# una-dinosauria/local-search-quantization

Hardware: AMD Instinct MI355X
Metric: vectors encoded/sec (ICM, m=8 h=256) (higher is better)
Workload: dtype f32

## Files before the change

### local-search-quantization_amd/csrc/lsq_icm.hip

```cpp
#include <stdlib.h>

#include <mutex>
#include <type_traits>

#include "lsq_wave.h"
#include "lsq_xload.h"
#include <atomic>

namespace {

template <int M, int SL, int ABL = 0, int DEPTH = 2, int NT = 1024>
__global__ __launch_bounds__(NT) void icm_walk_kernel(const float *__restrict__ U, const float *__restrict__ Ts, const float *__restrict__ T,
                                                        uint8_t *__restrict__ rec, unsigned short *__restrict__ valid,
                                                        int64_t n, const WalkNodes nodes, int per_pass, int use_skip, int direct_max,
                                                        unsigned long long *__restrict__ active_total,
                                                        const uint8_t *__restrict__ ref_rec, const unsigned short *__restrict__ ref_valid,
                                                        const int *__restrict__ idle_if_set) {
    constexpr int CS = (M <= 8) ? 8 : 16;
    constexpr int NS = LSQ_H / SL;
    if (idle_if_set && *idle_if_set) return;
    constexpr int LPV = SL / 4;
    constexpr int VPW = 64 / LPV;
    constexpr int CW = (M - 1 + 3) / 4;
    constexpr int RW = CS / 4;
// ... 140 lines not shown
            try_phase(std::integral_constant<int, 0>{}); try_phase(std::integral_constant<int, 1>{});
            try_phase(std::integral_constant<int, 2>{}); try_phase(std::integral_constant<int, 3>{});
            try_phase(std::integral_constant<int, 4>{}); try_phase(std::integral_constant<int, 5>{});
            try_phase(std::integral_constant<int, 6>{}); try_phase(std::integral_constant<int, 7>{});
        }
        __syncthreads();
    };

    const int64_t npass = (n + per_pass - 1) / per_pass;
    for (int64_t pass = blockIdx.x; pass < npass; pass += gridDim.x) {
        const int64_t lo = pass * per_pass;
        const int64_t hi = (lo + per_pass < n) ? lo + per_pass : n;
        const int cnt = (int)(hi - lo);

        for (int nu = 0; nu < nodes.count; ++nu) {
        const int j = nodes.j[nu];
        const float *__restrict__ Usj = U + (int64_t)j * n * LSQ_H;
        {
            const int base = (int)threadIdx.x * EPT;
            int f[EPT], c = 0;
#pragma unroll
            for (int e = 0; e < EPT; ++e) {
                const int idx = base + e;
                f[e] = 0;
                if (idx < cnt) f[e] = (!use_skip) || !((valid[lo + idx] >> j) & 1);
                c += f[e];
            }
            int inc = c;
#pragma unroll
            for (int off = 1; off < 64; off <<= 1) {
                const int t = __shfl_up(inc, off, 64);
                if (lane >= off) inc += t;
            }
            if (lane == 63) wave_tot[wave] = inc;
            __syncthreads();
            int wbase = 0;
            for (int w2 = 0; w2 < wave; ++w2) wbase += wave_tot[w2];
            int pos = wbase + inc - c;
#pragma unroll
            for (int e = 0; e < EPT; ++e)
                if (f[e]) list[pos++] = (unsigned short)(base + e);
            if (threadIdx.x == NT - 1) nact_s = wbase + inc;
            __syncthreads();
        }
        const int nact = nact_s;
        if (nact == 0) { __syncthreads(); continue; }
        if (threadIdx.x == 0) {
            stat_s[0] += (unsigned)nact;
            stat_s[nact <= direct_max ? 2 : 1] += 1u;
            stat_s[4 + ((nodes.pos0 + nu) & (LSQ_WALK_TRACE - 1))] += (unsigned)nact;
        }
        if (nact <= direct_max) {
            const float *__restrict__ Tj = T + (int64_t)j * M * LSQ_H * LSQ_H;
            constexpr int LB = LSQ_LIGHT_LB(M);
            for (int r0 = wave; r0 < nact; r0 += NW * LB) {
                int64_t vi[LB];
                bool on[LB];
#pragma unroll
                for (int e = 0; e < LB; ++e) {
                    const int r = r0 + e * NW;
                    on[e] = r < nact;
                    vi[e] = lo + __builtin_amdgcn_readfirstlane((int)list[on[e] ? r : r0]);
                }
                light_update<M, CS, LB>(rec, valid, ref_rec, ref_valid, Usj, Tj, n, SL, j, vi, on, lane);
            }
            __syncthreads();
            continue;
        }
        for (int ci = threadIdx.x; ci < nact; ci += NT) best64[ci] = ~0ull;

        walk_slices(j, lo, nact, nact == cnt, 0, NS);
        {
            constexpr int EPD = (PP + NT - 1) / NT;
            int64_t vi[EPD];
            uint32_t vcode[EPD];
            bool von[EPD];
#pragma unroll
            for (int e = 0; e < EPD; ++e) {
                const int ci = (int)threadIdx.x + e * NT;
                von[e] = ci < nact;
                vi[e] = lo + (von[e] ? list[ci] : 0);
                vcode[e] = von[e] ? (uint32_t)(best64[ci] & 0xffffffffull) : 0u;
            }
            apply_node_results<CS, EPD>(rec, valid, vi, vcode, von, j, ref_rec, ref_valid);
        }
        __syncthreads();
        }
    }
    __syncthreads();
    if (active_total)
        for (int e = threadIdx.x; e < 4 + LSQ_WALK_TRACE; e += NT)
            if (stat_s[e]) atomicAdd(active_total + e, (unsigned long long)stat_s[e]);
}

template <int SL>
__global__ __launch_bounds__(256) void tables_to_slices_kernel(const float *__restrict__ T, float *__restrict__ Ts, int m) {
    constexpr int NS = LSQ_H / SL, LPV = SL / 4;
    const int64_t total = (int64_t)m * NS * (m - 1) * LSQ_H * LPV;
    const int64_t e = (int64_t)blockIdx.x * 256 + threadIdx.x;
    if (e >= total) return;
    const int qq = (int)(e % LPV);
    int64_t r = e / LPV;
    const int b = (int)(r % LSQ_H); r /= LSQ_H;
    const int kk = (int)(r % (m - 1)); r /= (m - 1);
    const int slice = (int)(r % NS);
    const int j = (int)(r / NS);
    const int k = kk + (kk >= j ? 1 : 0);
    reinterpret_cast<f32x4 *>(Ts)[e] =
        *reinterpret_cast<const f32x4 *>(T + (((int64_t)j * m + k) * LSQ_H + b) * LSQ_H + slice * SL + qq * 4);
}

template <int M>
__global__ __launch_bounds__(256) void icm_wave_kernel(const float *__restrict__ U, const float *__restrict__ T, uint8_t *__restrict__ rec,
                                                       unsigned short *__restrict__ valid, int64_t n, const WalkNodes nodes, int SL, int use_skip,
                                                       unsigned long long *__restrict__ active_total, const uint8_t *__restrict__ ref_rec,
                                                       const unsigned short *__restrict__ ref_valid, const int *__restrict__ idle_if_set) {
    constexpr int CS = (M <= 8) ? 8 : 16;
    constexpr int LB = LSQ_LIGHT_LB(M);
    if (idle_if_set && *idle_if_set) return;
    __shared__ unsigned stat_s[4 + LSQ_WALK_TRACE];
    for (int e = threadIdx.x; e < 4 + LSQ_WALK_TRACE; e += 256) stat_s[e] = 0u;
    __syncthreads();
    const int lane = threadIdx.x & 63;
    const int64_t wv = (int64_t)blockIdx.x * 4 + __builtin_amdgcn_readfirstlane((int)(threadIdx.x >> 6));
    const int64_t i0 = wv * LB;
    const int LPV = SL / 4;
    const bool have_ref = ref_rec && ref_valid;
    CodeRec cr[LB], rr[LB];
    uint32_t vm[LB], rv[LB];
    bool on[LB];
#pragma unroll
    for (int e = 0; e < LB; ++e) {
        on[e] = i0 + e < n;
        cr[e].lo = cr[e].hi = rr[e].lo = rr[e].hi = 0ull;
        vm[e] = rv[e] = 0u;
        if (on[e]) {
            cr[e] = load_rec<CS>(rec, i0 + e);
            if (valid) vm[e] = (uint32_t)__builtin_amdgcn_readfirstlane((int)valid[i0 + e]);
            if (have_ref) {
                rr[e] = load_rec<CS>(ref_rec, i0 + e);
                rv[e] = (uint32_t)__builtin_amdgcn_readfirstlane((int)ref_valid[i0 + e]);
            }
        }
    }
    unsigned total = 0, wave_nodes = 0;
    for (int nu = 0; nu < nodes.count; ++nu) {
        const int j = nodes.j[nu];
        bool need[LB];
        unsigned cnt = 0;
#pragma unroll
        for (int e = 0; e < LB; ++e) {
            need[e] = on[e] && (!use_skip || !((vm[e] >> j) & 1u));
            cnt += need[e] ? 1u : 0u;
        }
        if (cnt == 0) continue;
        const float *__restrict__ Usj = U + (int64_t)j * n * LSQ_H;
        const float *__restrict__ Tj = T + (int64_t)j * M * LSQ_H * LSQ_H;
        f32x4 s[LB], c[LB][M > 1 ? M - 1 : 1];
#pragma unroll
        for (int e = 0; e < LB; ++e) {
            s[e] = (f32x4){0.f, 0.f, 0.f, 0.f};
            if (need[e]) s[e] = (reinterpret_cast<const f32x4 *>(Usj + ((int64_t)(lane / LPV) * n + (i0 + e)) * SL))[lane % LPV];
        }
#pragma unroll
        for (int e = 0; e < LB; ++e)
            if (need[e]) {
#pragma unroll
                for (int kk = 0; kk < M - 1; ++kk) {
                    const int k = kk + (kk >= j ? 1 : 0);
                    c[e][kk] = reinterpret_cast<const f32x4 *>(Tj + ((int64_t)(k * LSQ_H) + cr[e].get(k)) * LSQ_H)[lane];
                }
            }
#pragma unroll
        for (int e = 0; e < LB; ++e)
            if (need[e]) {
#pragma unroll
                for (int kk = 0; kk < M - 1; ++kk) s[e] = s[e] + c[e][kk];
                const uint32_t code = (uint32_t)wave_first_argmin(s[e], lane);
                if (code != cr[e].get(j)) { cr[e].set(j, code); vm[e] = 1u << j; }
                else vm[e] |= 1u << j;
                if (have_ref && cr[e].lo == rr[e].lo && (CS == 8 || cr[e].hi == rr[e].hi)) vm[e] |= rv[e];
            }
        total += cnt;
        ++wave_nodes;
        if (lane == 0) atomicAdd(&stat_s[4 + ((nodes.pos0 + nu) & (LSQ_WALK_TRACE - 1))], cnt);
    }
#pragma unroll
    for (int e = 0; e < LB; ++e)
        if (on[e] && lane == 0) {
            *reinterpret_cast<uint64_t *>(rec + (i0 + e) * CS) = cr[e].lo;
            if (CS == 16) *reinterpret_cast<uint64_t *>(rec + (i0 + e) * CS + 8) = cr[e].hi;
            if (valid) valid[i0 + e] = (unsigned short)vm[e];
        }
    if (lane == 0) { atomicAdd(&stat_s[0], total); atomicAdd(&stat_s[2], wave_nodes); }
    __syncthreads();
    if (active_total)
        for (int e = threadIdx.x; e < 4 + LSQ_WALK_TRACE; e += 256)
            if (stat_s[e]) atomicAdd(active_total + e, (unsigned long long)stat_s[e]);
}

__device__ inline bool perturb_record(uint64_t (&w)[2], int m, int npert, uint64_t seed, uint32_t it, uint64_t gi) {
    int need = npert < m ? npert : m;
    bool changed = false;
    for (int g = 0; 4 * g < m && need > 0; ++g) {
        const lsq_u32x4 sel = lsq_rng_block(seed, gi, it, LSQ_DOM_PERTURB, (uint32_t)g);
        const lsq_u32x4 vals = lsq_rng_block(seed, gi, it, LSQ_DOM_PERTURB, (uint32_t)(4 + g));
#pragma unroll
        for (int e = 0; e < 4; ++e) {
            const int pp = 4 * g + e;
            if (pp < m && need > 0 && lsq_mulhi32(sel.v[e], (uint32_t)(m - pp)) < (uint32_t)need) {
                const uint64_t val = lsq_mulhi32(vals.v[e], LSQ_H);
                const int sh = 8 * (pp & 7);
                changed |= (((w[pp >> 3] >> sh) & 0xffull) != val);
                w[pp >> 3] = (w[pp >> 3] & ~(0xffull << sh)) | (val << sh);
                --need;
            }
        }
    }
    return changed;
}

template <int CS>
__device__ inline void perturb_next_store(const lsq_perturb_next &pn, int64_t i, const uint32_t (&fin)[CS / 4], unsigned short vfin) {
    uint64_t w[2];
    w[0] = (uint64_t)fin[0] | ((uint64_t)fin[1] << 32);
    w[1] = (CS == 16) ? ((uint64_t)fin[CS / 4 - 2] | ((uint64_t)fin[CS / 4 - 1] << 32)) : 0ull;
#ifdef LSQ_TUNING
    if (pn.abl & 16) return;
    const bool changed = (pn.abl & 1) ? false : perturb_record(w, pn.m, pn.npert, pn.seed, pn.it, pn.goff + (uint64_t)i);
#else
    const bool changed = perturb_record(w, pn.m, pn.npert, pn.seed, pn.it, pn.goff + (uint64_t)i);
#endif
    uint64_t *q = reinterpret_cast<uint64_t *>(pn.dst + i * CS);
    q[0] = w[0];
    if (CS == 16) q[1] = w[1];
    if (pn.vdst) pn.vdst[i] = changed ? (unsigned short)0 : vfin;
}

template <int CS>
__global__ __launch_bounds__(256) void perturb_kernel(const uint8_t *__restrict__ src, uint8_t *__restrict__ dst, int64_t n,
                                                      int m, int npert, uint64_t seed, uint32_t it, uint64_t goff,
                                                      const unsigned short *__restrict__ vsrc, unsigned short *__restrict__ vdst) {
    const int64_t i = (int64_t)blockIdx.x * blockDim.x + threadIdx.x;
    if (i >= n) return;
    uint64_t w[2];
    const uint64_t *p = reinterpret_cast<const uint64_t *>(src + i * CS);
    w[0] = p[0];
    w[1] = (CS == 16) ? p[1] : 0ull;
    const bool changed = perturb_record(w, m, npert, seed, it, goff + (uint64_t)i);
    uint64_t *q = reinterpret_cast<uint64_t *>(dst + i * CS);
    q[0] = w[0];
    if (CS == 16) q[1] = w[1];
    if (vdst) vdst[i] = changed ? (unsigned short)0 : vsrc[i];
}

template <int VW>
__device__ inline int load_start(int c, int lp, int s) { return c + 16 * VW * s + VW * lp; }
template <int VW, typename OFF>
__device__ inline f32x4 load4(const float *p, OFF off, int c, int lp, int d) {
    if constexpr (VW == 4) {
        const int t = load_start<VW>(c, lp, 0);
        return *reinterpret_cast<const f32x4 *>(p + (size_t)(off + (OFF)(t < d ? t : 0)));
    }
    f32x4 v;
#pragma unroll
    for (int s = 0; s < 4; ++s) {
        const int t = load_start<VW>(c, lp, s);
        v[s] = p[(size_t)(off + (OFF)(t < d ? t : 0))];
    }
    return v;
}

template <class XT, int VW> struct XQuad { f32x4 v; __device__ f32x4 get() const { return v; } };
template <> struct XQuad<uint8_t, 4> { uint32_t w; __device__ f32x4 get() const { return lsq_widen4(w); } };
template <> struct XQuad<uint8_t, 1> {
    uint32_t b[4];
    __device__ f32x4 get() const { return (f32x4){(float)b[0], (float)b[1], (float)b[2], (float)b[3]}; }
};
template <int VW>
__device__ inline XQuad<float, VW> xquad_load(const float *x, int c, int lp, int d) { return XQuad<float, VW>{load4<VW>(x, 0, c, lp, d)}; }
template <int VW>
__device__ inline XQuad<uint8_t, VW> xquad_load(const uint8_t *x, int c, int lp, int d) {
    XQuad<uint8_t, VW> q;
    if constexpr (VW == 4) {
        const int t = load_start<VW>(c, lp, 0);
        q.w = lsq_ld4_packed(x + (t < d ? t : 0));
    } else {
#pragma unroll
        for (int s = 0; s < 4; ++s) {
            const int t = load_start<VW>(c, lp, s);
            q.b[s] = x[t < d ? t : 0];
        }
    }
    return q;
}

__device__ inline float row_sum16(float v) {
    v = v + dpp_self<DPP_XOR1, 0xf>(v);
    v = v + dpp_self<DPP_XOR2, 0xf>(v);
    v = v + dpp_self<DPP_HALF_MIRROR, 0xf>(v);
    return v + dpp_self<DPP_MIRROR, 0xf>(v);
}

template <int M, int MODE, int HASV, int NQ, int VW, class XT = float>
__device__ inline void cost4_body(const XT *__restrict__ X, const float *__restrict__ K,
                                  const uint8_t *rec, uint8_t *cur, float *__restrict__ prev,
                                  unsigned long long *__restrict__ counters, int64_t n, int64_t w, int64_t nwaves, int d,
                                  const unsigned short *vnew, unsigned short *vcur, const lsq_perturb_next &pn) {
    static_assert(VW == 4 || VW == 1, "load width: 16 or 4 bytes");
    using koff_t = std::conditional_t<VW == 4, uint32_t, uint64_t>;
    constexpr int CS = (M <= 8) ? 8 : 16;
    constexpr int RW = CS / 4;
    const int lane = threadIdx.x & 63;
    const int qtr = lane >> 4, lp = lane & 15;
    unsigned n_eq = 0, n_lt = 0;
    for (int64_t base = w * 64; base < n; base += nwaves * 64) {
        const int64_t il = base + lane;
        const bool livel = il < n;
        const int64_t ic = livel ? il : n - 1;
        uint32_t rn[RW], cw[RW];
        float pl = 0.0f;
        unsigned short vc = 0, vn = 0;
        {
            const uint32_t *rp = reinterpret_cast<const uint32_t *>(rec + ic * CS), *cp = reinterpret_cast<const uint32_t *>(cur + ic * CS);
#pragma unroll
            for (int q = 0; q < RW; ++q) rn[q] = rp[q];
            if (MODE == 1) {
#pragma unroll
                for (int q = 0; q < RW; ++q) cw[q] = cp[q];
                pl = prev[ic];
            }
            if (HASV) vc = vcur[ic];
            if (HASV && MODE == 1) vn = vnew[ic];
        }
        bool same = (MODE == 1);
#pragma unroll
        for (int q = 0; q < RW; ++q) {
            if (MODE == 0) cw[q] = rn[q];
            same = same && (rn[q] == cw[q]);
        }
        const bool skip = livel && same && (pl == pl);
        const unsigned nskip = (unsigned)__popcll(__ballot(skip));
        if (lane == 0) n_eq += nskip;
        unsigned short vfin = vc;
        const bool merge_v = HASV && MODE == 1 && same && livel;
        if (merge_v) vfin = (unsigned short)(vfin | vn);
        uint64_t accepted = 0;
        float newp = 0.0f;
        uint64_t todo = __ballot(livel && !skip);
#ifdef LSQ_TUNING
        if (pn.abl & 8) todo = 0;
#endif
        int nsidx[4];
        bool nhv[4];
        auto pick = [&]() {
#pragma unroll
            for (int v = 0; v < 4; ++v) {
                nhv[v] = todo != 0;
                nsidx[v] = nhv[v] ? __builtin_ctzll(todo) : (v ? nsidx[0] : 0);
                if (nhv[v]) todo &= todo - 1;
            }
        };
        auto xrow = [&]() -> const XT * {
            const int mys = qtr == 0 ? nsidx[0] : qtr == 1 ? nsidx[1] : qtr == 2 ? nsidx[2] : nsidx[3];
            return X + (base + mys) * (int64_t)d;
        };
        XQuad<XT, VW> xn[NQ];
        auto xload = [&](const XT *x, int c0) {
#pragma unroll
            for (int g = 0; g < NQ; ++g) {
                xn[g] = xquad_load<VW>(x, c0 + 64 * g, lp, d);
            }
        };
        pick();
        const XT *xnext = xrow();
        if (nhv[0]) xload(xnext, 0);
        while (nhv[0]) {
            int sidx[4];
            bool hv[4];
#pragma unroll
            for (int v = 0; v < 4; ++v) { sidx[v] = nsidx[v]; hv[v] = nhv[v]; }
            const XT *x = xnext;
            pick();
            xnext = xrow();
            const bool live = qtr == 0 ? hv[0] : qtr == 1 ? hv[1] : qtr == 2 ? hv[2] : hv[3];
            uint32_t r[RW];
            float pc;
            {
                uint32_t rv4[4][RW];
                float pc4[4];
#pragma unroll
                for (int v = 0; v < 4; ++v) {
#pragma unroll
                    for (int q = 0; q < RW; ++q) rv4[v][q] = (uint32_t)__builtin_amdgcn_readlane((int)rn[q], sidx[v]);
                    pc4[v] = __int_as_float(__builtin_amdgcn_readlane(__float_as_int(pl), sidx[v]));
                }
#pragma unroll
                for (int q = 0; q < RW; ++q) r[q] = qtr == 0 ? rv4[0][q] : qtr == 1 ? rv4[1][q] : qtr == 2 ? rv4[2][q] : rv4[3][q];
                pc = qtr == 0 ? pc4[0] : qtr == 1 ? pc4[1] : qtr == 2 ? pc4[2] : pc4[3];
            }
            koff_t kb[M];
#pragma unroll
            for (int k = 0; k < M; ++k) kb[k] = ((koff_t)(k * LSQ_H) + (koff_t)((r[k >> 2] >> (8 * (k & 3))) & 0xffu)) * (koff_t)d;
            f32x4 p = (f32x4){0.f, 0.f, 0.f, 0.f};
            for (int c0 = 0; c0 < d; c0 += 64 * NQ) {
                f32x4 xv[NQ], kv[NQ][M];
                bool ok[NQ][4];
#pragma unroll
                for (int g = 0; g < NQ; ++g) {
                    const int c = c0 + 64 * g;
#pragma unroll
                    for (int e = 0; e < 4; ++e) ok[g][e] = load_start<VW>(c, lp, e / VW) < d;
                    xv[g] = xn[g].get();
#pragma unroll
                    for (int k = 0; k < M; ++k) kv[g][k] = load4<VW>(K, kb[k], c, lp, d);
                }
                if (c0 + 64 * NQ < d) xload(x, c0 + 64 * NQ);
                else xload(xnext, 0);
#pragma unroll
                for (int g = 0; g < NQ; ++g) {
                    f32x4 cb = (f32x4){0.f, 0.f, 0.f, 0.f};
#pragma unroll
                    for (int k = 0; k < M; ++k) cb = cb + kv[g][k];
                    const f32x4 rr = cb - xv[g];
                    const f32x4 sq = rr * rr;
                    p.x = p.x + (ok[g][0] ? sq.x : 0.0f);
                    p.y = p.y + (ok[g][1] ? sq.y : 0.0f);
                    p.z = p.z + (ok[g][2] ? sq.z : 0.0f);
                    p.w = p.w + (ok[g][3] ? sq.w : 0.0f);
                }
            }
            float cost;
            if constexpr (VW == 4) cost = row_sum16((p.x + p.y) + (p.z + p.w));
            else cost = (row_sum16(p.x) + row_sum16(p.y)) + (row_sum16(p.z) + row_sum16(p.w));
#pragma unroll
            for (int v2 = 0; v2 < 4; ++v2) {
                const float cv = __int_as_float(__builtin_amdgcn_readlane(__float_as_int(cost), 16 * v2));
                if (hv[v2] && lane == sidx[v2]) newp = cv;
            }
            if (MODE == 1) {
                const bool eq = live && (cost == pc), lt = live && (cost < pc);
                const uint64_t bl = __ballot(lt && lp == 0);
                const unsigned ne = (unsigned)__popcll(__ballot(eq && lp == 0)), nl = (unsigned)__popcll(bl);
#pragma unroll
                for (int v2 = 0; v2 < 4; ++v2)
                    if ((bl >> (16 * v2)) & 1ull) accepted |= 1ull << sidx[v2];
                if (lane == 0) { n_eq += ne; n_lt += nl; }
            }
        }
        const bool acc = (accepted >> lane) & 1ull;
        if (MODE == 0) {
            if (livel) prev[il] = newp;
        } else if (acc) {
            prev[il] = newp;
            uint32_t *qd = reinterpret_cast<uint32_t *>(cur + il * CS);
#pragma unroll
            for (int q = 0; q < RW; ++q) qd[q] = rn[q];
        }
        if (HASV && MODE == 1 && (acc || merge_v)) vcur[il] = acc ? vn : vfin;
        if (pn.on && livel) {
            uint32_t fin[RW];
#pragma unroll
            for (int q = 0; q < RW; ++q) fin[q] = acc ? rn[q] : cw[q];
            perturb_next_store<CS>(pn, il, fin, acc ? vn : vfin);
        }
    }
    if (MODE == 1) {
        __shared__ unsigned cnt_s[2];
        if (threadIdx.x == 0) { cnt_s[0] = 0u; cnt_s[1] = 0u; }
        __syncthreads();
        if (lane == 0 && n_eq) atomicAdd(&cnt_s[0], n_eq);
        if (lane == 0 && n_lt) atomicAdd(&cnt_s[1], n_lt);
        __syncthreads();
        if (threadIdx.x == 0 && cnt_s[0]) atomicAdd(&counters[0], (unsigned long long)cnt_s[0]);
        if (threadIdx.x == 0 && cnt_s[1]) atomicAdd(&counters[1], (unsigned long long)cnt_s[1]);
    }
}

template <int M, int MODE, int HASV, int NQ, int VW, class XT = float>
__global__ __launch_bounds__(256) void cost4_kernel(const XT *__restrict__ X, const float *__restrict__ K, const uint8_t *rec, uint8_t *cur,
                                                    float *__restrict__ prev, unsigned long long *__restrict__ counters, int64_t n, int d,
                                                    const unsigned short *vnew, unsigned short *vcur, const lsq_perturb_next pn) {
    cost4_body<M, MODE, HASV, NQ, VW, XT>(X, K, rec, cur, prev, counters, n, __builtin_amdgcn_readfirstlane((int)(blockIdx.x * 4 + (threadIdx.x >> 6))),
                                      (int64_t)gridDim.x * 4, d, vnew, vcur, pn);
}
template <int M, int MODE, int HASV, int NQ, int VW, class XT = float>
__global__ __launch_bounds__(256) __attribute__((amdgpu_waves_per_eu(4, 4))) void cost4w_kernel(const XT *__restrict__ X, const float *__restrict__ K,
                                                    const uint8_t *rec, uint8_t *cur, float *__restrict__ prev,
                                                    unsigned long long *__restrict__ counters, int64_t n, int d,
                                                    const unsigned short *vnew, unsigned short *vcur, const lsq_perturb_next pn) {
    cost4_body<M, MODE, HASV, NQ, VW, XT>(X, K, rec, cur, prev, counters, n, __builtin_amdgcn_readfirstlane((int)(blockIdx.x * 4 + (threadIdx.x >> 6))),
                                      (int64_t)gridDim.x * 4, d, vnew, vcur, pn);
}

__global__ __launch_bounds__(256) void sum_f64_kernel(const float *__restrict__ v, int64_t n, double *__restrict__ sum) {
    __shared__ double sh[4];
    double acc = 0.0;
    for (int64_t i = (int64_t)blockIdx.x * blockDim.x + threadIdx.x; i < n; i += (int64_t)gridDim.x * blockDim.x) acc += (double)v[i];
    for (int off = 32; off > 0; off >>= 1) acc += __shfl_down(acc, off, 64);
    if ((threadIdx.x & 63) == 0) sh[threadIdx.x >> 6] = acc;
    __syncthreads();
    if (threadIdx.x == 0) atomicAdd(sum, sh[0] + sh[1] + sh[2] + sh[3]);
}

template <int CS>
__global__ __launch_bounds__(256) void codes_expand_kernel(const uint8_t *__restrict__ tight, int64_t n, int m, uint8_t *__restrict__ rec) {
    const int64_t i = (int64_t)blockIdx.x * blockDim.x + threadIdx.x;
    if (i >= n) return;
    uint64_t w[2] = {0ull, 0ull};
    for (int j = 0; j < m; ++j) w[j >> 3] |= (uint64_t)tight[i * m + j] << (8 * (j & 7));
    uint64_t *q = reinterpret_cast<uint64_t *>(rec + i * CS);
    q[0] = w[0];
    if (CS == 16) q[1] = w[1];
}
template <int CS>
__global__ __launch_bounds__(256) void codes_compact_kernel(const uint8_t *__restrict__ rec, int64_t n, int m, uint8_t *__restrict__ tight) {
    const int64_t i = (int64_t)blockIdx.x * blockDim.x + threadIdx.x;
    if (i >= n) return;
    for (int j = 0; j < m; ++j) tight[i * m + j] = rec[i * CS + j];
}
template <int CS>
__global__ __launch_bounds__(256) void codes_from_i16_kernel(const int16_t *__restrict__ B, int64_t n, int m, int h,
                                                             uint8_t *__restrict__ rec, int *__restrict__ bad) {
    const int64_t i = (int64_t)blockIdx.x * blockDim.x + threadIdx.x;
    if (i >= n) return;
    uint64_t w[2] = {0ull, 0ull};
    for (int j = 0; j < m; ++j) {
        const int v = (int)B[i * m + j];
        if (v < 1 || v > h) { *bad = 1; continue; }
        w[j >> 3] |= (uint64_t)(v - 1) << (8 * (j & 7));
    }
    uint64_t *q = reinterpret_cast<uint64_t *>(rec + i * CS);
    q[0] = w[0];
    if (CS == 16) q[1] = w[1];
}
template <int CS>
__global__ __launch_bounds__(256) void codes_to_i16_kernel(const uint8_t *__restrict__ rec, int64_t n, int m, int16_t *__restrict__ B) {
    const int64_t i = (int64_t)blockIdx.x * blockDim.x + threadIdx.x;
    if (i >= n) return;
    for (int j = 0; j < m; ++j) B[i * m + j] = (int16_t)(rec[i * CS + j] + 1);
}

__global__ __launch_bounds__(256) void synth_data_u8_kernel(uint64_t seed, uint64_t goff, int64_t n, int d, float *__restrict__ X) {
    const int64_t q = (int64_t)blockIdx.x * blockDim.x + threadIdx.x;
    const int d4 = (d + 3) >> 2;
    if (q >= n * d4) return;
    const int64_t i = q / d4;
    const int t0 = (int)(q % d4) * 4;
    const lsq_u32x4 r = lsq_rng_block(seed, goff + (uint64_t)i, (uint32_t)(t0 >> 10), LSQ_DOM_DATA, (uint32_t)((t0 & 1023) >> 2));
    for (int e = 0; e < 4 && t0 + e < d; ++e) X[i * (int64_t)d + t0 + e] = (float)(r.v[e] >> 24);
}
__global__ __launch_bounds__(256) void randinit_kernel(uint64_t seed, uint64_t goff, int64_t n, int m, int h, uint8_t *__restrict__ tight) {
    const int64_t i = (int64_t)blockIdx.x * blockDim.x + threadIdx.x;
    if (i >= n) return;
    for (int j = 0; j < m; ++j)
        tight[i * m + j] = (uint8_t)lsq_mulhi32(lsq_rng_word(seed, goff + (uint64_t)i, 0, LSQ_DOM_INIT, (uint32_t)j), (uint32_t)h);
}
__global__ __launch_bounds__(256) void synth_codebooks_kernel(uint64_t seed, int m, int h, int d, float *__restrict__ K) {
    const int64_t q = (int64_t)blockIdx.x * blockDim.x + threadIdx.x;
    if (q >= (int64_t)m * h * d) return;
    const int64_t row = q / d;
    const int t = (int)(q % d);
    const uint64_t pick = lsq_rng_word(seed, (uint64_t)row, 0, LSQ_DOM_CODEBOOK, 0);
    const uint32_t w = lsq_rng_word(seed ^ 0x5bd1e995ull, pick, (uint32_t)(t >> 10), LSQ_DOM_DATA, (uint32_t)(t & 1023));
    K[q] = (float)(w >> 24) / (float)m;
}

inline unsigned thread_grid(int64_t n) { return (unsigned)((n + 255) / 256); }

}


template <int M, int SL, int ABL = 0, int DEPTH = 2, int NT = 1024>
static int launch_walk_t(hipStream_t s, const float *U, const float *Ts, const float *T, uint8_t *rec, unsigned short *valid, int64_t n,
                         const WalkNodes &nodes, int use_skip, unsigned long long *active_total, int light,
                         const uint8_t *ref_rec, const unsigned short *ref_valid, const int *idle_if_set) {
    constexpr int TAB = (M - 1) * LSQ_H * (SL / 4);
    constexpr int PP = lsq_walk_pp(M, SL);
    constexpr int LDS_BYTES = TAB * 16 + PP * 8 + PP * 2;
    static_assert(LDS_BYTES + 256 <= 160 * 1024, "slice table + running best must fit the 160 KiB LDS");
    int per_pass = 1, npass = 1;
    lsq_walk_geometry(n, PP, &per_pass, &npass);
    const int direct_max = light >= 0 ? light : LSQ_KNOB("LSQ_WALK_DIRECT", 256);
    const int skip = (use_skip && valid) ? 1 : 0;
    static LdsOptIn optin;
    LSQ_TRY(optin_lds(optin, &icm_walk_kernel<M, SL, ABL, DEPTH, NT>, LDS_BYTES));
    const unsigned grid = (unsigned)(npass < 256 ? npass : 256);
    hipLaunchKernelGGL((icm_walk_kernel<M, SL, ABL, DEPTH, NT>), dim3(grid), dim3(NT), LDS_BYTES, s, U, Ts, T, rec, valid, n, nodes, per_pass,
                       skip, (T && ABL == 0) ? direct_max : 0, active_total, skip ? ref_rec : nullptr, skip ? ref_valid : nullptr, idle_if_set);
    LSQ_HIP(hipGetLastError());
    return LSQ_OK;
}

int lsq_launch_icm_walk(hipStream_t s, const float *U, const float *Ts, const float *T, uint8_t *rec, unsigned short *valid, int64_t n, int m,
                        const int32_t *order, int nnodes, int pos0, int max_per, int use_skip, unsigned long long *active_total, int ablation, int light,
                        const uint8_t *ref_rec, const unsigned short *ref_valid, const int *idle_if_set, int *launched) {
    if (n <= 0 || nnodes <= 0) return LSQ_OK;
    return for_walk_launches(order, nnodes, pos0, m, max_per, launched, [&](const WalkNodes &nodes) -> int {
#define LSQ_WALK_ARGS s, U, Ts, T, rec, valid, n, nodes, use_skip, active_total, light, ref_rec, ref_valid, idle_if_set
#define LSQ_WALK_CASE_MID(MM) case MM: LSQ_TRY((launch_walk_t<MM, 8, 0, 2>(LSQ_WALK_ARGS))); break;
#define LSQ_WALK_CASE_BIG(MM) case MM: LSQ_TRY((launch_walk_t<MM, 8, 0, 4, 512>(LSQ_WALK_ARGS))); break;
#define LSQ_WALK_CASE(MM) case MM: LSQ_TRY((launch_walk_t<MM, 16, 0, 3>(LSQ_WALK_ARGS))); break;
#ifdef LSQ_TUNING
        if (m == 8 && ablation == 1) return launch_walk_t<8, 16, 1>(LSQ_WALK_ARGS);
        if (m == 8 && ablation == 2) return launch_walk_t<8, 16, 2>(LSQ_WALK_ARGS);
        if (m == 8 && ablation == 3) return launch_walk_t<8, 16, 3>(LSQ_WALK_ARGS);
        if (m == 8 && ablation == 4) return launch_walk_t<8, 16, 4>(LSQ_WALK_ARGS);
#else
        (void)ablation;
#endif
        switch (m) {
            LSQ_WALK_CASE(1) LSQ_WALK_CASE(2) LSQ_WALK_CASE(3) LSQ_WALK_CASE(4)
            LSQ_WALK_CASE(5) LSQ_WALK_CASE(6) LSQ_WALK_CASE(7) LSQ_WALK_CASE(8)
            LSQ_WALK_CASE_MID(9) LSQ_WALK_CASE_MID(10) LSQ_WALK_CASE_MID(11) LSQ_WALK_CASE_MID(12)
            LSQ_WALK_CASE_MID(13) LSQ_WALK_CASE_BIG(14) LSQ_WALK_CASE_BIG(15) LSQ_WALK_CASE_BIG(16)
        }
#undef LSQ_WALK_ARGS
#undef LSQ_WALK_CASE
#undef LSQ_WALK_CASE_BIG
#undef LSQ_WALK_CASE_MID
        return LSQ_OK;
    });
}

int lsq_launch_tables_to_slices(hipStream_t s, const float *T, float *Ts, int m, int sl) {
    if (m < 2) return LSQ_OK;
    const int64_t total = (int64_t)m * (LSQ_H / sl) * (m - 1) * LSQ_H * (sl / 4);
    const unsigned grid = (unsigned)((total + 255) / 256);
    if (sl == 16) hipLaunchKernelGGL(tables_to_slices_kernel<16>, dim3(grid), dim3(256), 0, s, T, Ts, m);
    else hipLaunchKernelGGL(tables_to_slices_kernel<8>, dim3(grid), dim3(256), 0, s, T, Ts, m);
    LSQ_HIP(hipGetLastError());
    return LSQ_OK;
}

#define LSQ_CS_LAUNCH(m, KERNEL, GRID, ...)                                                       \
    do {                                                                                           \
        if (lsq_code_stride(m) == 8) hipLaunchKernelGGL(KERNEL<8>, dim3(GRID), dim3(256), 0, s, __VA_ARGS__);  \
        else hipLaunchKernelGGL(KERNEL<16>, dim3(GRID), dim3(256), 0, s, __VA_ARGS__);             \
        LSQ_HIP(hipGetLastError());                                                                \
    } while (0)

int lsq_launch_icm_wave(hipStream_t s, const float *U, const float *T, uint8_t *rec, unsigned short *valid, int64_t n, int m, const int32_t *order,
                        int nnodes, int pos0, int max_per, int use_skip, unsigned long long *active_total, const uint8_t *ref_rec,
                        const unsigned short *ref_valid, int *launched) {
    if (n <= 0 || nnodes <= 0) return LSQ_OK;
    const int skip = (use_skip && valid) ? 1 : 0;
    LSQ_TRY(for_walk_launches(order, nnodes, pos0, m, max_per, launched, [&](const WalkNodes &nodes) -> int {
        const int lb = LSQ_LIGHT_LB(m);
        const unsigned grid = (unsigned)((n + 4 * lb - 1) / (4 * lb));
        LSQ_DISPATCH_M(m, hipLaunchKernelGGL(icm_wave_kernel<M_>, dim3(grid), dim3(256), 0, s, U, T, rec, valid, n, nodes, lsq_walk_slice_width(m), skip,
                                             active_total, skip ? ref_rec : nullptr, skip ? ref_valid : nullptr, static_cast<const int *>(nullptr)));
        return LSQ_OK;
    }));
    LSQ_HIP(hipGetLastError());
    return LSQ_OK;
}

int lsq_launch_perturb(hipStream_t s, const uint8_t *src, uint8_t *dst, int64_t n, int m, int npert, uint64_t seed,
                       uint32_t it, uint64_t global_offset, const unsigned short *vsrc, unsigned short *vdst) {
    if (n <= 0) return LSQ_OK;
    LSQ_CS_LAUNCH(m, perturb_kernel, thread_grid(n), src, dst, n, m, npert, seed, it, global_offset, vsrc, vdst);
    return LSQ_OK;
}

const void *lsq_probe_kernel_icm() { return reinterpret_cast<const void *>(&tables_to_slices_kernel<16>); }

template <int M, int NQ, int VW, class XT>
static void launch_cost_t(hipStream_t s, const XT *X, const float *K, const uint8_t *rec, uint8_t *cur, float *prev,
                          unsigned long long *counters, int64_t n, int d, int mode, const unsigned short *vnew, unsigned short *vcur,
                          const lsq_perturb_next &pn) {
    static std::atomic<int> per_cu_known[3];
    auto launch = [&](auto kern, int which) {
        int per_cu = per_cu_known[which].load(std::memory_order_relaxed);
        if (per_cu == 0) {
            int nb = 0;
            if (hipOccupancyMaxActiveBlocksPerMultiprocessor(&nb, kern, 256, 0) != hipSuccess || nb < 1) nb = 4;
            per_cu = nb > 8 ? 8 : nb;
            per_cu_known[which].store(per_cu, std::memory_order_relaxed);
        }
        const int64_t want = (n + 255) / 256, cap = 256 * (int64_t)per_cu;
        hipLaunchKernelGGL(kern, dim3((unsigned)(want < cap ? want : cap)), dim3(256), 0, s, X, K, rec, cur, prev, counters, n, d, vnew, vcur, pn);
    };
    if constexpr (NQ == 1) {
        if (mode == 1) launch(cost4_kernel<M, 1, 1, 1, VW, XT>, 0); else if (vcur) launch(cost4_kernel<M, 0, 1, 1, VW, XT>, 1); else launch(cost4_kernel<M, 0, 0, 1, VW, XT>, 2);
    } else if constexpr (M <= 8) {
        if (mode == 1) launch(cost4w_kernel<M, 1, 1, 2, VW, XT>, 0); else if (vcur) launch(cost4w_kernel<M, 0, 1, 2, VW, XT>, 1); else launch(cost4w_kernel<M, 0, 0, 2, VW, XT>, 2);
    }
}

template <class XT>
static int launch_cost_x(hipStream_t s, const XT *X, const float *K, const uint8_t *rec, uint8_t *cur, float *prev,
                         unsigned long long *counters, int64_t n, int d, int m, int mode, const unsigned short *vnew, unsigned short *vcur,
                         const lsq_perturb_next *next) {
    if (n <= 0) return LSQ_OK;
    if (mode == 1 && (!vnew || !vcur)) { lsq_set_error("lsq_launch_cost: accept mode needs both validity arrays"); return LSQ_EINVAL; }
    lsq_perturb_next pn = {};
    if (next) pn = *next;
    pn.abl = LSQ_KNOB("LSQ_COST_ABL", 0);
    if (d % 4 == 0 && lsq_x_vec_ok(X) && (uintptr_t)K % 16 == 0) {
        if ((int64_t)m * LSQ_H * d >= (1ll << 31)) { lsq_set_error("lsq_launch_cost: codebook matrix too large"); return LSQ_EINVAL; }
        if (d > 64 && m <= 8) {
            LSQ_DISPATCH_M(m, (launch_cost_t<M_, 2, 4>(s, X, K, rec, cur, prev, counters, n, d, mode, vnew, vcur, pn)));
        } else {
            LSQ_DISPATCH_M(m, (launch_cost_t<M_, 1, 4>(s, X, K, rec, cur, prev, counters, n, d, mode, vnew, vcur, pn)));
        }
    } else {
        LSQ_DISPATCH_M(m, (launch_cost_t<M_, 1, 1>(s, X, K, rec, cur, prev, counters, n, d, mode, vnew, vcur, pn)));
    }
    LSQ_HIP(hipGetLastError());
    return LSQ_OK;
}

int lsq_launch_cost(hipStream_t s, const float *X, const float *K, const uint8_t *rec, uint8_t *cur, float *prev,
                    unsigned long long *counters, int64_t n, int d, int m, int mode, const unsigned short *vnew, unsigned short *vcur,
                    const lsq_perturb_next *next) {
    return launch_cost_x(s, X, K, rec, cur, prev, counters, n, d, m, mode, vnew, vcur, next);
}
int lsq_launch_cost(hipStream_t s, const uint8_t *X, const float *K, const uint8_t *rec, uint8_t *cur, float *prev,
                    unsigned long long *counters, int64_t n, int d, int m, int mode, const unsigned short *vnew, unsigned short *vcur,
                    const lsq_perturb_next *next) {
    return launch_cost_x(s, X, K, rec, cur, prev, counters, n, d, m, mode, vnew, vcur, next);
}

int lsq_launch_sum_f64(hipStream_t s, const float *v, int64_t n, double *sum) {
    if (n <= 0) return LSQ_OK;
    unsigned g = thread_grid(n);
    if (g > 1024) g = 1024;
    hipLaunchKernelGGL(sum_f64_kernel, dim3(g), dim3(256), 0, s, v, n, sum);
    LSQ_HIP(hipGetLastError());
    return LSQ_OK;
}

int lsq_launch_codes_expand(hipStream_t s, const uint8_t *tight, int64_t n, int m, uint8_t *rec) {
    if (n <= 0) return LSQ_OK;
    LSQ_CS_LAUNCH(m, codes_expand_kernel, thread_grid(n), tight, n, m, rec);
    return LSQ_OK;
}
int lsq_launch_codes_compact(hipStream_t s, const uint8_t *rec, int64_t n, int m, uint8_t *tight) {
    if (n <= 0) return LSQ_OK;
    LSQ_CS_LAUNCH(m, codes_compact_kernel, thread_grid(n), rec, n, m, tight);
    return LSQ_OK;
}
int lsq_launch_codes_from_i16(hipStream_t s, const int16_t *B, int64_t n, int m, int h, uint8_t *rec, int *bad_flag) {
    if (n <= 0) return LSQ_OK;
    LSQ_CS_LAUNCH(m, codes_from_i16_kernel, thread_grid(n), B, n, m, h, rec, bad_flag);
    return LSQ_OK;
}
int lsq_launch_codes_to_i16(hipStream_t s, const uint8_t *rec, int64_t n, int m, int16_t *B) {
    if (n <= 0) return LSQ_OK;
    LSQ_CS_LAUNCH(m, codes_to_i16_kernel, thread_grid(n), rec, n, m, B);
    return LSQ_OK;
}

int lsq_launch_synth_data_u8(hipStream_t s, uint64_t seed, uint64_t global_offset, int64_t n, int d, float *X) {
    if (n <= 0) return LSQ_OK;
    const int64_t items = n * ((d + 3) >> 2);
    hipLaunchKernelGGL(synth_data_u8_kernel, dim3(thread_grid(items)), dim3(256), 0, s, seed, global_offset, n, d, X);
    LSQ_HIP(hipGetLastError());
    return LSQ_OK;
}
int lsq_launch_randinit(hipStream_t s, uint64_t seed, uint64_t global_offset, int64_t n, int m, int h, uint8_t *tight) {
    if (n <= 0) return LSQ_OK;
    hipLaunchKernelGGL(randinit_kernel, dim3(thread_grid(n)), dim3(256), 0, s, seed, global_offset, n, m, h, tight);
    LSQ_HIP(hipGetLastError());
    return LSQ_OK;
}
int lsq_launch_synth_codebooks(hipStream_t s, uint64_t seed, int m, int h, int d, float *K) {
    hipLaunchKernelGGL(synth_codebooks_kernel, dim3(thread_grid((int64_t)m * h * d)), dim3(256), 0, s, seed, m, h, d, K);
    LSQ_HIP(hipGetLastError());
    return LSQ_OK;
}
```

Baseline: 21.36 million.

## Add software-pipelined buffer-load cost kernel for m<=8 with cross-row prefetch

Replaces the NQ=2 cost kernel for m<=8 with a new body that uses raw buffer loads with out-of-bounds clamping in place of per-lane bounds checks. It double-buffers codeword and X quads across 64-column chunks and across row groups, and prefetches the next batch's codes, prev costs and validity words while the current batch computes. The aim is to hide memory latency and remove address and predicate arithmetic, at the cost of higher register pressure and more complex control flow. It also applies to d<=64, and shared pre-load and store helpers are factored out.

Result: no change. 21.53 million, median of 2 (+0.8%).

```diff
diff --git a/local-search-quantization_amd/csrc/lsq_icm.hip b/local-search-quantization_amd/csrc/lsq_icm.hip
--- a/local-search-quantization_amd/csrc/lsq_icm.hip
+++ b/local-search-quantization_amd/csrc/lsq_icm.hip
@@ -466,7 +466,66 @@
     return v + dpp_self<DPP_MIRROR, 0xf>(v);
 }
 
-template <int M, int MODE, int HASV, int NQ, int VW, class XT = float>
+template <int RW>
+struct CostPre { uint32_t rn[RW], cw[RW]; float pl; unsigned short vc, vn; };
+template <int RW, int MODE, int HASV>
+__device__ inline void cost_pre_load(CostPre<RW> &q, const uint8_t *rec, const uint8_t *cur, const float *prev, const unsigned short *vnew,
+                                     const unsigned short *vcur, int64_t ic) {
+    const uint32_t *rp = reinterpret_cast<const uint32_t *>(rec + ic * (4 * RW)), *cp = reinterpret_cast<const uint32_t *>(cur + ic * (4 * RW));
+    q.pl = 0.0f;
+    q.vc = 0;
+    q.vn = 0;
+#pragma unroll
+    for (int e = 0; e < RW; ++e) q.rn[e] = rp[e];
+#pragma unroll
+    for (int e = 0; e < RW; ++e) q.cw[e] = (MODE == 1) ? cp[e] : q.rn[e];
+    if (MODE == 1) q.pl = prev[ic];
+    if (HASV) q.vc = vcur[ic];
+    if (HASV && MODE == 1) q.vn = vnew[ic];
+}
+template <int RW, int MODE, int HASV>
+__device__ inline void cost_batch_store(const CostPre<RW> &q, bool livel, int64_t il, bool acc, bool merge_v, unsigned short vfin, float newp,
+                                        uint8_t *cur, float *prev, unsigned short *vcur, const lsq_perturb_next &pn) {
+    if (MODE == 0) {
+        if (livel) prev[il] = newp;
+    } else if (acc) {
+        prev[il] = newp;
+        uint32_t *qd = reinterpret_cast<uint32_t *>(cur + il * (4 * RW));
+#pragma unroll
+        for (int e = 0; e < RW; ++e) qd[e] = q.rn[e];
+    }
+    if (HASV && MODE == 1 && (acc || merge_v)) vcur[il] = acc ? q.vn : vfin;
+    if (pn.on && livel) {
+        uint32_t fin[RW];
+#pragma unroll
+        for (int e = 0; e < RW; ++e) fin[e] = acc ? q.rn[e] : q.cw[e];
+        perturb_next_store<4 * RW>(pn, il, fin, acc ? q.vn : vfin);
+    }
+}
+template <int M>
+__device__ inline void cost_step_add(f32x4 &p, const f32x4 (&kv)[M], f32x4 xv, const bool (&ok)[4]) {
+    f32x4 cb = (f32x4){0.f, 0.f, 0.f, 0.f};
+#pragma unroll
+    for (int k = 0; k < M; ++k) cb = cb + kv[k];
+    const f32x4 rr = cb - xv;
+    const f32x4 sq = rr * rr;
+    p.x = p.x + (ok[0] ? sq.x : 0.0f);
+    p.y = p.y + (ok[1] ? sq.y : 0.0f);
+    p.z = p.z + (ok[2] ? sq.z : 0.0f);
+    p.w = p.w + (ok[3] ? sq.w : 0.0f);
+}
+__device__ inline void cost_counters_add(unsigned long long *counters, int lane, unsigned n_eq, unsigned n_lt) {
+    __shared__ unsigned cnt_s[2];
+    if (threadIdx.x == 0) { cnt_s[0] = 0u; cnt_s[1] = 0u; }
+    __syncthreads();
+    if (lane == 0 && n_eq) atomicAdd(&cnt_s[0], n_eq);
+    if (lane == 0 && n_lt) atomicAdd(&cnt_s[1], n_lt);
+    __syncthreads();
+    if (threadIdx.x == 0 && cnt_s[0]) atomicAdd(&counters[0], (unsigned long long)cnt_s[0]);
+    if (threadIdx.x == 0 && cnt_s[1]) atomicAdd(&counters[1], (unsigned long long)cnt_s[1]);
+}
+
+template <int M, int MODE, int HASV, int VW, class XT = float>
 __device__ inline void cost4_body(const XT *__restrict__ X, const float *__restrict__ K,
                                   const uint8_t *rec, uint8_t *cur, float *__restrict__ prev,
                                   unsigned long long *__restrict__ counters, int64_t n, int64_t w, int64_t nwaves, int d,
@@ -482,27 +541,14 @@
         const int64_t il = base + lane;
         const bool livel = il < n;
         const int64_t ic = livel ? il : n - 1;
-        uint32_t rn[RW], cw[RW];
-        float pl = 0.0f;
-        unsigned short vc = 0, vn = 0;
-        {
-            const uint32_t *rp = reinterpret_cast<const uint32_t *>(rec + ic * CS), *cp = reinterpret_cast<const uint32_t *>(cur + ic * CS);
-#pragma unroll
-            for (int q = 0; q < RW; ++q) rn[q] = rp[q];
-            if (MODE == 1) {
-#pragma unroll
-                for (int q = 0; q < RW; ++q) cw[q] = cp[q];
-                pl = prev[ic];
-            }
-            if (HASV) vc = vcur[ic];
-            if (HASV && MODE == 1) vn = vnew[ic];
-        }
+        CostPre<RW> pr;
+        cost_pre_load<RW, MODE, HASV>(pr, rec, cur, prev, vnew, vcur, ic);
+        const uint32_t (&rn)[RW] = pr.rn;
+        const float pl = pr.pl;
+        const unsigned short vc = pr.vc, vn = pr.vn;
         bool same = (MODE == 1);
 #pragma unroll
-        for (int q = 0; q < RW; ++q) {
-            if (MODE == 0) cw[q] = rn[q];
-            same = same && (rn[q] == cw[q]);
-        }
+        for (int q = 0; q < RW; ++q) same = same && (rn[q] == pr.cw[q]);
         const bool skip = livel && same && (pl == pl);
         const unsigned nskip = (unsigned)__popcll(__ballot(skip));
         if (lane == 0) n_eq += nskip;
@@ -529,13 +575,8 @@
             const int mys = qtr == 0 ? nsidx[0] : qtr == 1 ? nsidx[1] : qtr == 2 ? nsidx[2] : nsidx[3];
             return X + (base + mys) * (int64_t)d;
         };
-        XQuad<XT, VW> xn[NQ];
-        auto xload = [&](const XT *x, int c0) {
-#pragma unroll
-            for (int g = 0; g < NQ; ++g) {
-                xn[g] = xquad_load<VW>(x, c0 + 64 * g, lp, d);
-            }
-        };
+        XQuad<XT, VW> xn;
+        auto xload = [&](const XT *x, int c0) { xn = xquad_load<VW>(x, c0, lp, d); };
         pick();
         const XT *xnext = xrow();
         if (nhv[0]) xload(xnext, 0);
@@ -567,32 +608,17 @@
 #pragma unroll
             for (int k = 0; k < M; ++k) kb[k] = ((koff_t)(k * LSQ_H) + (koff_t)((r[k >> 2] >> (8 * (k & 3))) & 0xffu)) * (koff_t)d;
             f32x4 p = (f32x4){0.f, 0.f, 0.f, 0.f};
-            for (int c0 = 0; c0 < d; c0 += 64 * NQ) {
-                f32x4 xv[NQ], kv[NQ][M];
-                bool ok[NQ][4];
-#pragma unroll
-                for (int g = 0; g < NQ; ++g) {
-                    const int c = c0 + 64 * g;
-#pragma unroll
-                    for (int e = 0; e < 4; ++e) ok[g][e] = load_start<VW>(c, lp, e / VW) < d;
-                    xv[g] = xn[g].get();
-#pragma unroll
-                    for (int k = 0; k < M; ++k) kv[g][k] = load4<VW>(K, kb[k], c, lp, d);
-                }
-                if (c0 + 64 * NQ < d) xload(x, c0 + 64 * NQ);
+            for (int c0 = 0; c0 < d; c0 += 64) {
+                f32x4 kv[M];
+                bool ok[4];
+#pragma unroll
+                for (int e = 0; e < 4; ++e) ok[e] = load_start<VW>(c0, lp, e / VW) < d;
+                const f32x4 xv = xn.get();
+#pragma unroll
+                for (int k = 0; k < M; ++k) kv[k] = load4<VW>(K, kb[k], c0, lp, d);
+                if (c0 + 64 < d) xload(x, c0 + 64);
                 else xload(xnext, 0);
-#pragma unroll
-                for (int g = 0; g < NQ; ++g) {
-                    f32x4 cb = (f32x4){0.f, 0.f, 0.f, 0.f};
-#pragma unroll
-                    for (int k = 0; k < M; ++k) cb = cb + kv[g][k];
-                    const f32x4 rr = cb - xv[g];
-                    const f32x4 sq = rr * rr;
-                    p.x = p.x + (ok[g][0] ? sq.x : 0.0f);
-                    p.y = p.y + (ok[g][1] ? sq.y : 0.0f);
-                    p.z = p.z + (ok[g][2] ? sq.z : 0.0f);
-                    p.w = p.w + (ok[g][3] ? sq.w : 0.0f);
-                }
+                cost_step_add<M>(p, kv, xv, ok);
             }
             float cost;
             if constexpr (VW == 4) cost = row_sum16((p.x + p.y) + (p.z + p.w));
@@ -612,49 +638,188 @@
                 if (lane == 0) { n_eq += ne; n_lt += nl; }
             }
         }
-        const bool acc = (accepted >> lane) & 1ull;
-        if (MODE == 0) {
-            if (livel) prev[il] = newp;
-        } else if (acc) {
-            prev[il] = newp;
-            uint32_t *qd = reinterpret_cast<uint32_t *>(cur + il * CS);
-#pragma unroll
-            for (int q = 0; q < RW; ++q) qd[q] = rn[q];
-        }
-        if (HASV && MODE == 1 && (acc || merge_v)) vcur[il] = acc ? vn : vfin;
-        if (pn.on && livel) {
-            uint32_t fin[RW];
-#pragma unroll
-            for (int q = 0; q < RW; ++q) fin[q] = acc ? rn[q] : cw[q];
-            perturb_next_store<CS>(pn, il, fin, acc ? vn : vfin);
-        }
-    }
-    if (MODE == 1) {
-        __shared__ unsigned cnt_s[2];
-        if (threadIdx.x == 0) { cnt_s[0] = 0u; cnt_s[1] = 0u; }
-        __syncthreads();
-        if (lane == 0 && n_eq) atomicAdd(&cnt_s[0], n_eq);
-        if (lane == 0 && n_lt) atomicAdd(&cnt_s[1], n_lt);
-        __syncthreads();
-        if (threadIdx.x == 0 && cnt_s[0]) atomicAdd(&counters[0], (unsigned long long)cnt_s[0]);
-        if (threadIdx.x == 0 && cnt_s[1]) atomicAdd(&counters[1], (unsigned long long)cnt_s[1]);
-    }
-}
-
-template <int M, int MODE, int HASV, int NQ, int VW, class XT = float>
+        cost_batch_store<RW, MODE, HASV>(pr, livel, il, (accepted >> lane) & 1ull, merge_v, vfin, newp, cur, prev, vcur, pn);
+    }
+    if (MODE == 1) cost_counters_add(counters, lane, n_eq, n_lt);
+}
+
+constexpr uint32_t COST_OOB = 0x40000000u;
+__device__ inline __amdgpu_buffer_rsrc_t cost_rsrc(const void *p, uint32_t bytes) {
+    return __builtin_amdgcn_make_buffer_rsrc(const_cast<void *>(p), 0, (int)bytes, 0x00020000);
+}
+__device__ inline void xquad_bufload(XQuad<float, 4> &q, __amdgpu_buffer_rsrc_t r, uint32_t off) {
+    q.v = __builtin_bit_cast(f32x4, __builtin_amdgcn_raw_buffer_load_b128(r, (int)off, 0, 0));
+}
+__device__ inline void xquad_bufload(XQuad<uint8_t, 4> &q, __amdgpu_buffer_rsrc_t r, uint32_t off) {
+    q.w = __builtin_amdgcn_raw_buffer_load_b32(r, (int)off, 0, 0);
+}
+
+template <int M, int MODE, int HASV, class XT = float>
+__device__ inline void cost4p_body(const XT *__restrict__ X, const float *__restrict__ K,
+                                   const uint8_t *rec, uint8_t *cur, float *__restrict__ prev,
+                                   unsigned long long *__restrict__ counters, int64_t n, int64_t w, int64_t nwaves, int d,
+                                   const unsigned short *vnew, unsigned short *vcur, const lsq_perturb_next &pn) {
+    static_assert(M <= 8, "two units of M codeword quads have to fit 128 VGPRs");
+    constexpr int RW = 2;
+    struct Unit { XQuad<XT, 4> x; f32x4 kv[M]; };
+    const int lane = threadIdx.x & 63;
+    const int qtr = lane >> 4, lp = lane & 15;
+    const __amdgpu_buffer_rsrc_t kres = cost_rsrc(K, (uint32_t)(M * LSQ_H) * (uint32_t)d * 4u);
+    unsigned n_eq = 0, n_lt = 0;
+    CostPre<RW> nx;
+    auto prefetch = [&](int64_t nbase) {
+        const int64_t left = n - nbase;
+        const uint32_t nv = left < 0 ? 0u : left < 64 ? (uint32_t)left : 64u;
+        typedef uint32_t u32x2 __attribute__((ext_vector_type(2)));
+        const u32x2 rv = __builtin_amdgcn_raw_buffer_load_b64(cost_rsrc(rec + nbase * 8, nv * 8u), lane * 8, 0, 0);
+        nx.rn[0] = rv.x;
+        nx.rn[1] = rv.y;
+        nx.cw[0] = rv.x;
+        nx.cw[1] = rv.y;
+        nx.pl = 0.0f;
+        nx.vc = 0;
+        nx.vn = 0;
+        if (MODE == 1) {
+            const u32x2 cv = __builtin_amdgcn_raw_buffer_load_b64(cost_rsrc(cur + nbase * 8, nv * 8u), lane * 8, 0, 0);
+            nx.cw[0] = cv.x;
+            nx.cw[1] = cv.y;
+            nx.pl = __uint_as_float(__builtin_amdgcn_raw_buffer_load_b32(cost_rsrc(prev + nbase, nv * 4u), lane * 4, 0, 0));
+        }
+        if (HASV) nx.vc = __builtin_amdgcn_raw_buffer_load_b16(cost_rsrc(vcur + nbase, nv * 2u), lane * 2, 0, 0);
+        if (HASV && MODE == 1) nx.vn = __builtin_amdgcn_raw_buffer_load_b16(cost_rsrc(vnew + nbase, nv * 2u), lane * 2, 0, 0);
+    };
+    prefetch(w * 64);
+    for (int64_t base = w * 64; base < n; base += nwaves * 64) {
+        const int64_t il = base + lane;
+        const bool livel = il < n;
+        const CostPre<RW> pr = nx;
+        const float pl = pr.pl;
+        bool same = (MODE == 1);
+#pragma unroll
+        for (int q = 0; q < RW; ++q) same = same && (pr.rn[q] == pr.cw[q]);
+        const bool skip = livel && same && (pl == pl);
+        const unsigned nskip = (unsigned)__popcll(__ballot(skip));
+        if (lane == 0) n_eq += nskip;
+        unsigned short vfin = pr.vc;
+        const bool merge_v = HASV && MODE == 1 && same && livel;
+        if (merge_v) vfin = (unsigned short)(vfin | pr.vn);
+        uint64_t accepted = 0;
+        float newp = 0.0f;
+        uint64_t todo = __ballot(livel && !skip);
+#ifdef LSQ_TUNING
+        if (pn.abl & 8) todo = 0;
+#endif
+        if (todo == 0) {
+            prefetch(base + nwaves * 64);
+        } else {
+            const int64_t left = n - base;
+            const __amdgpu_buffer_rsrc_t xres = cost_rsrc(X + base * (int64_t)d, (uint32_t)(left < 64 ? left : 64) * (uint32_t)d * (uint32_t)sizeof(XT));
+            uint32_t ni = 0, si = 0;
+            int nrows = 0, srows = 0;
+            int smys = 0;
+            uint32_t rr[RW] = {0u, 0u}, xb = 0, spare = 0;
+            const uint32_t d4 = (uint32_t)d * 4u;
+            int ci = d, cs = 0;
+            int nmys = 0;
+            f32x4 p = (f32x4){0.f, 0.f, 0.f, 0.f};
+            bool more_left = true;
+            auto more = [&]() {
+                if (ci + 64 < d) { ci += 64; return; }
+                if (todo == 0) { more_left = false; return; }
+                ni = 0;
+                nrows = 0;
+#pragma unroll
+                for (int v = 0; v < 4; ++v)
+                    if (todo != 0) {
+                        ni |= (uint32_t)__builtin_ctzll(todo) << (8 * v);
+                        todo &= todo - 1;
+                        ++nrows;
+                    }
+                spare = qtr < nrows ? 0u : COST_OOB;
+                nmys = (int)((ni >> (8 * qtr)) & 0xffu) * 4;
+#pragma unroll
+                for (int q = 0; q < RW; ++q) rr[q] = (uint32_t)__builtin_amdgcn_ds_bpermute(nmys, (int)pr.rn[q]);
+                xb = __umul24((uint32_t)nmys, (uint32_t)d * (uint32_t)sizeof(XT) / 4u) + spare;
+                ci = 0;
+            };
+            auto issue = [&](Unit &u) {
+                const int t = ci + 4 * lp;
+                const bool in = t < d && more_left;
+                const uint32_t tk = (in ? (uint32_t)t * 4u : COST_OOB) + spare, tx = in ? (uint32_t)t * (uint32_t)sizeof(XT) : COST_OOB;
+                xquad_bufload(u.x, xres, xb + tx);
+#pragma unroll
+                for (int k = 0; k < M; ++k)
+                    u.kv[k] = __builtin_bit_cast(f32x4, __builtin_amdgcn_raw_buffer_load_b128(
+                                  kres, (int)(__umul24((rr[k >> 2] >> (8 * (k & 3))) & 0xffu, d4) + tk), (int)((uint32_t)(k * LSQ_H) * d4), 0));
+            };
+            auto sum = [&](const Unit &u) {
+                const bool in = cs + 4 * lp < d;
+                const bool ok[4] = {in, in, in, in};
+                cost_step_add<M>(p, u.kv, u.x.get(), ok);
+                cs += 64;
+            };
+            auto adopt = [&]() { si = ni; srows = nrows; smys = nmys; };
+            auto close = [&]() {
+                const float cost = row_sum16((p.x + p.y) + (p.z + p.w));
+#pragma unroll
+                for (int v = 0; v < 4; ++v) {
+                    const float cv = __int_as_float(__builtin_amdgcn_readlane(__float_as_int(cost), 16 * v));
+                    if (v < srows && lane == (int)((si >> (8 * v)) & 0xffu)) newp = cv;
+                }
+                if (MODE == 1) {
+                    const float pc = __int_as_float(__builtin_amdgcn_ds_bpermute(smys, __float_as_int(pl)));
+                    const bool live = qtr < srows;
+                    const bool eq = live && (cost == pc), lt = live && (cost < pc);
+                    const uint64_t bl = __ballot(lt && lp == 0);
+                    const unsigned ne = (unsigned)__popcll(__ballot(eq && lp == 0)), nl = (unsigned)__popcll(bl);
+#pragma unroll
+                    for (int v = 0; v < 4; ++v)
+                        if ((bl >> (16 * v)) & 1ull) accepted |= 1ull << ((si >> (8 * v)) & 0xffu);
+                    if (lane == 0) { n_eq += ne; n_lt += nl; }
+                }
+                p = (f32x4){0.f, 0.f, 0.f, 0.f};
+                cs = 0;
+                adopt();
+            };
+            Unit ua, ub;
+            more();
+            adopt();
+            issue(ua);
+            while (more_left) {
+                more();
+                const bool m1 = more_left;
+                issue(ub);
+                if (!m1) prefetch(base + nwaves * 64);
+                sum(ua);
+                if (cs >= d) close();
+                more();
+                issue(ua);
+                if (m1) {
+                    if (!more_left) prefetch(base + nwaves * 64);
+                    sum(ub);
+                    if (cs >= d) close();
+                }
+            }
+        }
+        cost_batch_store<RW, MODE, HASV>(pr, livel, il, (accepted >> lane) & 1ull, merge_v, vfin, newp, cur, prev, vcur, pn);
+    }
+    if (MODE == 1) cost_counters_add(counters, lane, n_eq, n_lt);
+}
+
+template <int M, int MODE, int HASV, int VW, class XT = float>
 __global__ __launch_bounds__(256) void cost4_kernel(const XT *__restrict__ X, const float *__restrict__ K, const uint8_t *rec, uint8_t *cur,
                                                     float *__restrict__ prev, unsigned long long *__restrict__ counters, int64_t n, int d,
                                                     const unsigned short *vnew, unsigned short *vcur, const lsq_perturb_next pn) {
-    cost4_body<M, MODE, HASV, NQ, VW, XT>(X, K, rec, cur, prev, counters, n, __builtin_amdgcn_readfirstlane((int)(blockIdx.x * 4 + (threadIdx.x >> 6))),
+    cost4_body<M, MODE, HASV, VW, XT>(X, K, rec, cur, prev, counters, n, __builtin_amdgcn_readfirstlane((int)(blockIdx.x * 4 + (threadIdx.x >> 6))),
                                       (int64_t)gridDim.x * 4, d, vnew, vcur, pn);
 }
-template <int M, int MODE, int HASV, int NQ, int VW, class XT = float>
+template <int M, int MODE, int HASV, class XT = float>
 __global__ __launch_bounds__(256) __attribute__((amdgpu_waves_per_eu(4, 4))) void cost4w_kernel(const XT *__restrict__ X, const float *__restrict__ K,
                                                     const uint8_t *rec, uint8_t *cur, float *__restrict__ prev,
                                                     unsigned long long *__restrict__ counters, int64_t n, int d,
                                                     const unsigned short *vnew, unsigned short *vcur, const lsq_perturb_next pn) {
-    cost4_body<M, MODE, HASV, NQ, VW, XT>(X, K, rec, cur, prev, counters, n, __builtin_amdgcn_readfirstlane((int)(blockIdx.x * 4 + (threadIdx.x >> 6))),
-                                      (int64_t)gridDim.x * 4, d, vnew, vcur, pn);
+    cost4p_body<M, MODE, HASV, XT>(X, K, rec, cur, prev, counters, n, __builtin_amdgcn_readfirstlane((int)(blockIdx.x * 4 + (threadIdx.x >> 6))),
+                                   (int64_t)gridDim.x * 4, d, vnew, vcur, pn);
 }
 
 __global__ __launch_bounds__(256) void sum_f64_kernel(const float *__restrict__ v, int64_t n, double *__restrict__ sum) {
@@ -829,7 +994,7 @@
 
 const void *lsq_probe_kernel_icm() { return reinterpret_cast<const void *>(&tables_to_slices_kernel<16>); }
 
-template <int M, int NQ, int VW, class XT>
+template <int M, bool PIPE, int VW, class XT>
 static void launch_cost_t(hipStream_t s, const XT *X, const float *K, const uint8_t *rec, uint8_t *cur, float *prev,
                           unsigned long long *counters, int64_t n, int d, int mode, const unsigned short *vnew, unsigned short *vcur,
                           const lsq_perturb_next &pn) {
@@ -845,10 +1010,10 @@
         const int64_t want = (n + 255) / 256, cap = 256 * (int64_t)per_cu;
         hipLaunchKernelGGL(kern, dim3((unsigned)(want < cap ? want : cap)), dim3(256), 0, s, X, K, rec, cur, prev, counters, n, d, vnew, vcur, pn);
     };
-    if constexpr (NQ == 1) {
-        if (mode == 1) launch(cost4_kernel<M, 1, 1, 1, VW, XT>, 0); else if (vcur) launch(cost4_kernel<M, 0, 1, 1, VW, XT>, 1); else launch(cost4_kernel<M, 0, 0, 1, VW, XT>, 2);
+    if constexpr (!PIPE) {
+        if (mode == 1) launch(cost4_kernel<M, 1, 1, VW, XT>, 0); else if (vcur) launch(cost4_kernel<M, 0, 1, VW, XT>, 1); else launch(cost4_kernel<M, 0, 0, VW, XT>, 2);
     } else if constexpr (M <= 8) {
-        if (mode == 1) launch(cost4w_kernel<M, 1, 1, 2, VW, XT>, 0); else if (vcur) launch(cost4w_kernel<M, 0, 1, 2, VW, XT>, 1); else launch(cost4w_kernel<M, 0, 0, 2, VW, XT>, 2);
+        if (mode == 1) launch(cost4w_kernel<M, 1, 1, XT>, 0); else if (vcur) launch(cost4w_kernel<M, 0, 1, XT>, 1); else launch(cost4w_kernel<M, 0, 0, XT>, 2);
     }
 }
 
@@ -863,13 +1028,13 @@
     pn.abl = LSQ_KNOB("LSQ_COST_ABL", 0);
     if (d % 4 == 0 && lsq_x_vec_ok(X) && (uintptr_t)K % 16 == 0) {
         if ((int64_t)m * LSQ_H * d >= (1ll << 31)) { lsq_set_error("lsq_launch_cost: codebook matrix too large"); return LSQ_EINVAL; }
-        if (d > 64 && m <= 8) {
-            LSQ_DISPATCH_M(m, (launch_cost_t<M_, 2, 4>(s, X, K, rec, cur, prev, counters, n, d, mode, vnew, vcur, pn)));
+        if (m <= 8 && (int64_t)m * LSQ_H * d * 4 <= (int64_t)COST_OOB) {
+            LSQ_DISPATCH_M(m, (launch_cost_t<M_, true, 4>(s, X, K, rec, cur, prev, counters, n, d, mode, vnew, vcur, pn)));
         } else {
-            LSQ_DISPATCH_M(m, (launch_cost_t<M_, 1, 4>(s, X, K, rec, cur, prev, counters, n, d, mode, vnew, vcur, pn)));
+            LSQ_DISPATCH_M(m, (launch_cost_t<M_, false, 4>(s, X, K, rec, cur, prev, counters, n, d, mode, vnew, vcur, pn)));
         }
     } else {
-        LSQ_DISPATCH_M(m, (launch_cost_t<M_, 1, 1>(s, X, K, rec, cur, prev, counters, n, d, mode, vnew, vcur, pn)));
+        LSQ_DISPATCH_M(m, (launch_cost_t<M_, false, 1>(s, X, K, rec, cur, prev, counters, n, d, mode, vnew, vcur, pn)));
     }
     LSQ_HIP(hipGetLastError());
     return LSQ_OK;
```
